# snphbaum/scikit-gpuppy

Measured on NVIDIA B200. Metric: fit_s_per_iter, lower is better.
Workload: dtype f64

## Files before the change

scikit-gpuppy_b200/csrc/gpk.cu:

```cuda
#include "../../include/gpk.h"
#include "../../include/gpk_test.h"

#include <climits>
#include <new>
#include <type_traits>
#include <vector>

#include "dgemm_dmma.cuh"
#include "factor.cuh"
#include "se_kernels.cuh"
#include "exact_kernels.cuh"
#include "periodic_kernels.cuh"

namespace gpk {
thread_local char g_err[512] = {0};
thread_local long g_launch_count = 0;
thread_local bool g_prof_on = false;
static thread_local std::vector<ProfPair> g_prof;
void prof_push(cudaEvent_t a, cudaEvent_t b) { g_prof.push_back(ProfPair{a, b}); }

struct Handle {
  int n = 0, d = 0, npad = 0;
  double *X = nullptr, *W = nullptr;
  bool own_X = false, own_W = false;
// ... 990 lines not shown
  if (npad % TILE) { snprintf(g_err, sizeof(g_err), "npad must be a multiple of 128"); return -2; }
  int* info_dev = nullptr;
  GPK_CUDA_OK(cudaMalloc((void**)&info_dev, sizeof(int)));
  set_int_kernel<<<1, 1, 0, st>>>(info_dev, INT_MAX);
  FactorCtx c{A, X, (long)ld, dL, info_dev, st};
  int rc = potrf_inv_node(c, 0, (int)npad);
  int info = 0;
  cudaError_t e = cudaMemcpyAsync(&info, info_dev, sizeof(int), cudaMemcpyDeviceToHost, st);
  if (e == cudaSuccess) e = cudaStreamSynchronize(st);
  cudaFree(info_dev);
  if (rc < 0) return rc;
  if (e != cudaSuccess) { snprintf(g_err, sizeof(g_err), "potrf_inv: %s", cudaGetErrorString(e)); return -1; }
  *info_host = (info == INT_MAX) ? 0 : info;
  return 0;
}

int gpk_test_oz_residues(const double* src, int64_t ld, int64_t rows, int64_t K, int trans, int lower, int moduli,
                         void* planes_out, double* scales_out, void* stream) {
  cudaStream_t st = reinterpret_cast<cudaStream_t>(stream);
  oz::Operand op;
  op.sl = reinterpret_cast<int8_t*>(planes_out); op.sc = scales_out;
  op.rows = (int)rows; op.K = (int)K; op.S = moduli;
  unsigned long long* mx = nullptr;
  GPK_CUDA_OK(cudaMalloc((void**)&mx, (size_t)rows * sizeof(unsigned long long)));
  int rc = oz::slice_operand(src, ld, trans, lower, op, mx, st);
  cudaError_t e = cudaStreamSynchronize(st);
  cudaFree(mx);
  if (rc < 0) return rc;
  if (e != cudaSuccess) { snprintf(g_err, sizeof(g_err), "oz_residues: %s", cudaGetErrorString(e)); return -1; }
  return 0;
}

int gpk_test_oz_gemm(const double* A, int64_t lda, int transA, int lowerA, const double* B, int64_t ldb, int transB,
                     int lowerB, double* C, int64_t ldc, int64_t M, int64_t N, int64_t K, double alpha, double beta,
                     int krange, int lower_only, int moduli, int64_t panel_rows, int reps, float* ms_out, void* stream) {
  cudaStream_t st = reinterpret_cast<cudaStream_t>(stream);
  oz::Operand a, b;
  a.rows = (int)M; a.K = (int)K; a.S = moduli;
  b.rows = (int)N; b.K = (int)K; b.S = moduli;
  unsigned long long* mx = nullptr;
  cudaEvent_t e0 = nullptr, e1 = nullptr, e2 = nullptr;
  int rc = 0;
  auto cleanup = [&]() {
    cudaFree(a.sl); cudaFree(a.sc); cudaFree(b.sl); cudaFree(b.sc); cudaFree(mx); cudaFree(a.out);
    if (e0) cudaEventDestroy(e0);
    if (e1) cudaEventDestroy(e1);
    if (e2) cudaEventDestroy(e2);
  };
#define OZ_OK(expr)                                                                         \
  do {                                                                                      \
    cudaError_t _e = (expr);                                                                \
    if (_e != cudaSuccess) {                                                                \
      snprintf(g_err, sizeof(g_err), "oz_gemm: %s -> %s", #expr, cudaGetErrorString(_e));   \
      cleanup();                                                                            \
      return -1;                                                                            \
    }                                                                                       \
  } while (0)
  OZ_OK(cudaMalloc((void**)&a.sl, oz::Operand::slice_bytes(a.rows, a.K, a.S)));
  OZ_OK(cudaMalloc((void**)&b.sl, oz::Operand::slice_bytes(b.rows, b.K, b.S)));
  OZ_OK(cudaMalloc((void**)&a.sc, (size_t)M * sizeof(double)));
  OZ_OK(cudaMalloc((void**)&b.sc, (size_t)N * sizeof(double)));
  OZ_OK(cudaMalloc((void**)&mx, (size_t)(M > N ? M : N) * sizeof(unsigned long long)));
  {
    const long prow = panel_rows > 0 ? round_up_l((long)panel_rows, 256) : round_up_l((long)M, 256);
    size_t want_out = (size_t)a.S * prow * round_up_l((long)N, 256);
    if (want_out > ((size_t)16 << 30)) want_out = (size_t)16 << 30;
    OZ_OK(cudaMalloc((void**)&a.out, want_out));
    a.out_cap = want_out;
  }
  OZ_OK(cudaEventCreate(&e0));
  OZ_OK(cudaEventCreate(&e1));
  OZ_OK(cudaEventCreate(&e2));
  OZ_OK(cudaEventRecord(e0, st));
  rc = oz::slice_operand(A, lda, transA, lowerA, a, mx, st);
  if (rc == 0) rc = oz::slice_operand(B, ldb, transB, lowerB, b, mx, st);
  if (rc < 0) { cleanup(); return rc; }
  OZ_OK(cudaEventRecord(e1, st));
  if (reps < 1) reps = 1;
  for (int r = 0; r < reps && rc == 0; ++r) rc = oz::gemm_sliced(a, b, C, ldc, alpha, beta, krange, lower_only, st);
  if (rc < 0) { cleanup(); return rc; }
  OZ_OK(cudaEventRecord(e2, st));
  OZ_OK(cudaStreamSynchronize(st));
  if (ms_out) {
    OZ_OK(cudaEventElapsedTime(&ms_out[0], e0, e1));
    OZ_OK(cudaEventElapsedTime(&ms_out[1], e1, e2));
    ms_out[1] /= reps;
  }
#undef OZ_OK
  cleanup();
  return 0;
}

int gpk_test_position_lock(int on) {
  if (on >= 0 && on <= 2) oz::g_position_lock = on;
  return oz::g_position_lock;
}

int gpk_test_overlap(int on) {
  if (on == 0 || on == 1) g_overlap_T = on;
  return g_overlap_T;
}

int gpk_profile(int on) {
  g_prof_on = on != 0;
  return 0;
}

int gpk_profile_read(double* gemm_ms, int64_t* gemm_launches, int64_t* all_launches, double* max_gemm_ms) {
  double total = 0.0, longest = 0.0;
  for (auto& p : g_prof) {
    float ms = 0.f;
    cudaError_t e = cudaEventSynchronize(p.b);
    if (e == cudaSuccess) e = cudaEventElapsedTime(&ms, p.a, p.b);
    cudaEventDestroy(p.a);
    cudaEventDestroy(p.b);
    if (e != cudaSuccess) {
      snprintf(g_err, sizeof(g_err), "gpk_profile_read: %s", cudaGetErrorString(e));
      g_prof.clear();
// ... 73 lines not shown
```

scikit-gpuppy_b200/csrc/oz_crt_planes.cuh:

```cuda

struct PlaneArgs {
  uint8_t* res; long res_ld; long res_plane;
  int M, N, K;
  int row_tile0;
  int krange, lower_only;
  int widen, band_cols;
  int nmod;
  unsigned int* phase;
  int* spill;
  int m[CRT_MAX_MODULI]; uint32_t magic[CRT_MAX_MODULI]; uint32_t u[CRT_MAX_MODULI];
};

constexpr int RECON_GROUPS = (CRT_MAX_MODULI + 3) / 4;

struct ReconArgs {
  const uint8_t* res; long res_ld; long res_plane;
  double* C; long ldc;
  const double* scA; const double* scB;
  double alpha, beta;
  int M, N, K;
  int row0;
  int krange, lower_only;
  int nmod;
  double p_scaled;
  double* colsq; double* pairdot; long ldo;
  uint32_t wp[2 * RECON_GROUPS][6];
};

constexpr int SPILL_SLOTS = 256;
constexpr int Q_BN = 256;
constexpr int Q_STAGES = 7;
constexpr int Q_STAGE_BYTES = 2 * TILE_BYTES;
constexpr int Q_SMEM_BYTES = Q_STAGES * Q_STAGE_BYTES + 1024 + 256;

__host__ __device__ __forceinline__ void planes_krange(int krange, int K, int bi2, int bx2, int& kb0, int& kb1) {
  kb0 = 0;
  kb1 = K / BK;
  switch (krange) {
    case K_UPTO_BJ: kb1 = (kb1 < 2 * bx2 + 2) ? kb1 : 2 * bx2 + 2; break;
    case K_FROM_BJ: kb0 = (kb1 < 2 * bx2) ? kb1 : 2 * bx2; break;
    case K_UPTO_BI: kb1 = (kb1 < 2 * bi2 + 2) ? kb1 : 2 * bi2 + 2; break;
    case K_FROM_BI: kb0 = (kb1 < 2 * bi2) ? kb1 : 2 * bi2; break;
    default: break;
  }
}

__global__ void __launch_bounds__(THREADS, 1)
// ... 24 lines not shown
    const int first = band * PLANES_BAND;
    const int cols = min(nx - first, PLANES_BAND);
    const int rem = pid - band * per_band;
    bx = first + rem % cols;
    by = rem / cols;
    band_lo = first;
    band_hi = first + cols - 1;
  }
  const int bi2 = by + p.row_tile0;
  const int bi = 2 * bi2 + pp;
  const int bjt = 2 * bx + pp;
  if (p.lower_only && 2 * bx > 2 * bi2 + 1) return;
  int kb0, kb1;
  planes_krange(p.krange, p.K, bi2, bx, kb0, kb1);
  if (kb1 <= kb0) return;
  if (p.widen) {
    const int kbt = p.K / BK;
    switch (p.krange) {
      case K_FROM_BI: case K_FROM_BJ: { const int u = min(kb0, 2 * band_lo); kb0 = max(u, kb0 - WIDEN_TILES); if (kb0 < 0) kb0 = 0; } break;
      case K_UPTO_BI: case K_UPTO_BJ: { const int u = max(kb1, min(kbt, 2 * band_hi + 2)); kb1 = min(u, kb1 + WIDEN_TILES); if (kb1 > kbt) kb1 = kbt; } break;
      default: break;
    }
  }
  const int nmod = p.nmod;

  const uint32_t raw = smem_u32(oz_smem_raw);
  uint8_t* smem = oz_smem_raw + ((1024u - (raw & 1023u)) & 1023u);
  uint64_t* bars = reinterpret_cast<uint64_t*>(smem + Q_STAGES * Q_STAGE_BYTES);
  uint64_t* full = bars;
  uint64_t* empty = bars + Q_STAGES;
  uint64_t* tmem_full = bars + 2 * Q_STAGES;
  uint64_t* tmem_empty = bars + 2 * Q_STAGES + 2;
  uint32_t* tmem_slot = reinterpret_cast<uint32_t*>(bars + 2 * Q_STAGES + 4);

  if (warp == 0 && lane == 0) {
    tma_prefetch_desc(&tmA);
    tma_prefetch_desc(&tmB);
  }
  if (warp == 1 && lane == 0) {
    for (int s = 0; s < Q_STAGES; ++s) {
      mbar_init(&full[s], 1);
      mbar_init(&empty[s], 1);
    }
    for (int b = 0; b < 2; ++b) {
      mbar_init(&tmem_full[b], 1);
      mbar_init(&tmem_empty[b], 2 * EPI_WARPS);
    }
// ... 71 lines not shown
            umma_i8_pair(acc, ad + (uint64_t)(k4 * 2), bd + (uint64_t)(k4 * 2), idesc, (kb > kbeg) | (k4 > 0));
          umma_commit_pair(&empty[stage], 3);
          if (++stage == Q_STAGES) { stage = 0; phase ^= 1u; }
        }
        umma_commit_pair(&tmem_full[buf], 3);
      }
    }
  } else {
    const int quad = warp & 3, half = (warp - 2) >> 2;
    const int row = quad * 32 + lane;
    const uint32_t lane_addr = tmem_base + ((uint32_t)(quad * 32) << 16);
    const long lrow = (long)by * (2 * BM) + pp * BM + row;
    uint8_t* dst0 = p.res + lrow * p.res_ld + (long)bx * Q_BN + half * 128;
    int4* sp = split ? reinterpret_cast<int4*>(p.spill + ((size_t)(smid % SPILL_SLOTS) * BM + row) * Q_BN + half * 128) : nullptr;
    for (int sg = 0; sg < nseg; ++sg) {
      const int i = SEG_MOD(sg);
      const bool spill_out = split && sg == 0, add_in = split && sg == nmod;
      const int buf = sg & 1;
      if (lane == 0) mbar_wait(&tmem_full[buf], (uint32_t)(sg >> 1) & 1u);
      __syncwarp();
      tc_fence_after();
      const int m = p.m[i];
      const int magic = (int)p.magic[i];
      const uint32_t u = p.u[i];
      uint8_t* dst = dst0 + (long)i * p.res_plane;
#pragma unroll
      for (int c = 0; c < 4; ++c) {
        uint32_t R[2][16];
        const uint32_t ta = lane_addr + (uint32_t)(buf * Q_BN + half * 128 + c * 32);
        tmem_ld16(ta, R[0]);
        tmem_ld16(ta + 16u, R[1]);
        tmem_ld_wait();
        if (c == 3) {
          tc_fence_before();
          __syncwarp();
          if (lane == 0) mbar_arrive_cluster(&tmem_empty[buf], rank & ~1u);
        }
        if (spill_out) {
#pragma unroll
          for (int x = 0; x < 8; ++x) {
            const uint32_t* r4 = &R[x >> 2][(x & 3) * 4];
            sp[c * 8 + x] = make_int4((int)r4[0], (int)r4[1], (int)r4[2], (int)r4[3]);
          }
          continue;
        }
        if (add_in) {
#pragma unroll
// ... 37 lines not shown
  uint32_t d;
  asm("dp2a.hi.u32.u32 %0, %1, %2, %3;" : "=r"(d) : "r"(a), "r"(b), "r"(c));
  return d;
}

template <int EPI, int NG>
__global__ void __launch_bounds__(256, 4) oz_crt_reconstruct_kernel(const __grid_constant__ ReconArgs p) {
  const int lane = threadIdx.x & 31, warp = threadIdx.x >> 5;
  const int bjc = blockIdx.x;
  const long lrow = (long)blockIdx.y * 8 + warp;
  const long grow = (long)p.row0 + lrow;
  const long gcol = (long)bjc * 128 + lane * 4;
  const int bi = (int)(grow >> 7), bi2 = (int)(grow >> 8), bx2 = bjc >> 1;
  if (EPI == OZ_EPI_STORE && p.lower_only && bjc > bi) return;
  int kb0, kb1;
  planes_krange(p.krange, p.K, bi2, bx2, kb0, kb1);
  const bool computed = (kb1 > kb0) && !(p.lower_only && 2 * bx2 > 2 * bi2 + 1);

  uint32_t acc[4][6];
#pragma unroll
  for (int x = 0; x < 4; ++x)
#pragma unroll
    for (int j = 0; j < 6; ++j) acc[x][j] = 0u;
  if (computed) {
    const uint8_t* src = p.res + lrow * p.res_ld + gcol;
    uint32_t q[NG * 4];
#pragma unroll
    for (int i = 0; i < NG * 4; ++i) {
      q[i] = (i < 4 * (NG - 1) || i < p.nmod) ? __ldcs(reinterpret_cast<const uint32_t*>(src)) : 0u;
      src += p.res_plane;
    }
#pragma unroll
    for (int g = 0; g < NG; ++g) {
      {
        const uint32_t ab_lo = __byte_perm(q[4 * g], q[4 * g + 1], 0x5140), ab_hi = __byte_perm(q[4 * g], q[4 * g + 1], 0x7362);
        const uint32_t cd_lo = __byte_perm(q[4 * g + 2], q[4 * g + 3], 0x5140),
                       cd_hi = __byte_perm(q[4 * g + 2], q[4 * g + 3], 0x7362);
        const uint32_t t[4] = {__byte_perm(ab_lo, cd_lo, 0x5410), __byte_perm(ab_lo, cd_lo, 0x7632),
                               __byte_perm(ab_hi, cd_hi, 0x5410), __byte_perm(ab_hi, cd_hi, 0x7632)};
#pragma unroll
        for (int e = 0; e < 4; ++e)
#pragma unroll
          for (int j = 0; j < 6; ++j) {
            uint32_t v = acc[e][j];
            v = dp2a_lo(p.wp[2 * g][j], t[e], v);
            v = dp2a_hi(p.wp[2 * g + 1][j], t[e], v);
            acc[e][j] = v;
          }
      }
    }
  }
  const bool row_ok = grow < p.M;
  const bool col_ok = gcol < p.N;
  const double sa = row_ok ? p.scA[grow] * p.p_scaled : 0.0;
  double v[4];
#pragma unroll
  for (int x = 0; x < 4; ++x) {
    const unsigned long long t0 = ((unsigned long long)acc[x][1] << 16) + acc[x][0];
    const unsigned long long t1 = ((unsigned long long)acc[x][3] << 16) + acc[x][2] + (t0 >> 32);
    const unsigned long long t2 = ((unsigned long long)acc[x][5] << 16) + acc[x][4] + (t1 >> 32);
    const long long hi = (long long)((t2 << 32) | (t1 & 0xffffffffull));
    const double frac = fma((double)hi, 4294967296.0, (double)(uint32_t)t0);
    v[x] = col_ok ? sa * p.scB[gcol + x] * frac : 0.0;
  }
  if (EPI == OZ_EPI_STORE) {
    if (row_ok && col_ok) {
      double* crow = p.C + grow * p.ldc + gcol;
#pragma unroll
      for (int x = 0; x < 4; x += 2) {
        double2 o;
        o.x = p.alpha * v[x];
        o.y = p.alpha * v[x + 1];
        if (p.beta != 0.0) {
          const double2 old = *reinterpret_cast<const double2*>(crow + x);
          o.x = fma(p.beta, old.x, o.x);
          o.y = fma(p.beta, old.y, o.y);
        }
// ... 26 lines not shown
```

scikit-gpuppy_b200/csrc/oz_gemm.cuh:

```cuda
#pragma once
#include <cuda.h>

#include "dgemm_dmma.cuh"
#include "oz_crt_tables.h"

namespace gpk {
namespace oz {

constexpr int BM = 128, BN = 128, BK = 128;
constexpr int TILE_BYTES = BM * BK;
constexpr int EPI_WARPS = 8;
constexpr int THREADS = 64 + EPI_WARPS * 32;
constexpr int TMEM_COLS = 512;

constexpr int OZ_EPI_STORE = 0;
constexpr int OZ_EPI_ROWSQ = 1;

__device__ __forceinline__ uint32_t smem_u32(const void* p) { return (uint32_t)__cvta_generic_to_shared(p); }

__device__ __forceinline__ void mbar_init(uint64_t* bar, uint32_t count) {
  asm volatile("mbarrier.init.shared::cta.b64 [%0], %1;" ::"r"(smem_u32(bar)), "r"(count) : "memory");
}
__device__ __forceinline__ void fence_barrier_init() {
  asm volatile("fence.mbarrier_init.release.cluster;" ::: "memory");
// ... 105 lines not shown

template <int TRANS>
__device__ __forceinline__ bool oz_valid(int r, int k, int lower) {
  if (!lower) return true;
  return TRANS ? ((r >> 7) <= (k >> 7)) : ((k >> 7) <= (r >> 7));
}
constexpr int WIDEN_MIN_K = 16384;
constexpr int PLANES_BAND = 4;
constexpr int WIDEN_TILES = 2 * (PLANES_BAND - 1);
inline int zero_fill_extra(int K) { return K >= WIDEN_MIN_K ? 1 + WIDEN_TILES : 1; }
template <int TRANS>
__device__ __forceinline__ bool oz_needed(int r, int k, int lower, int extra) {
  if (!lower) return true;
  return TRANS ? ((r >> 7) <= (k >> 7) + extra) : ((k >> 7) <= (r >> 7) + extra);
}

__device__ __forceinline__ size_t slice_offset(int rows, int K, int p, int r, int k) {
  const size_t tiles_per_plane = (size_t)(rows >> 7) * (size_t)(K >> 7);
  return (((size_t)p * tiles_per_plane + (size_t)(r >> 7) * (size_t)(K >> 7) + (size_t)(k >> 7)) << 14) +
         ((size_t)(r & 127) << 7) + (size_t)(k & 127);
}

__global__ void __launch_bounds__(256) oz_absmax_rows_kernel(const double* __restrict__ src, long ld, int K, int lower,
                                                             unsigned long long* __restrict__ mx) {
  __shared__ double red[8];
  const int r = blockIdx.x;
  const int kend = lower ? min(K, ((r >> 7) + 1) << 7) : K;
  const double* row = src + (long)r * ld;
  double m = 0.0;
  for (int k = threadIdx.x; k < kend; k += 256) m = fmax(m, fabs(row[k]));
#pragma unroll
  for (int o = 16; o > 0; o >>= 1) m = fmax(m, __shfl_xor_sync(0xffffffffu, m, o));
  if ((threadIdx.x & 31) == 0) red[threadIdx.x >> 5] = m;
  __syncthreads();
  if (threadIdx.x == 0) {
#pragma unroll
    for (int i = 0; i < 8; ++i) m = fmax(m, red[i]);
    mx[r] = (unsigned long long)__double_as_longlong(m);
  }
}
__global__ void __launch_bounds__(256) oz_absmax_cols_kernel(const double* __restrict__ src, long ld, int K, int lower,
                                                             unsigned long long* __restrict__ mx) {
  __shared__ double red[8][32];
  const int lane = threadIdx.x & 31, w = threadIdx.x >> 5;
  const int r = blockIdx.x * 32 + lane;
  const int k0 = blockIdx.y * 1024, k1 = min(K, k0 + 1024);
  const int kfirst = lower ? ((r >> 7) << 7) : 0;
  double m = 0.0;
  for (int k = k0 + w; k < k1; k += 8)
    if (k >= kfirst) m = fmax(m, fabs(src[(long)k * ld + r]));
  red[w][lane] = m;
  __syncthreads();
  if (w == 0) {
#pragma unroll
    for (int i = 1; i < 8; ++i) m = fmax(m, red[i][lane]);
    atomicMax(mx + r, (unsigned long long)__double_as_longlong(m));
  }
}

__device__ __forceinline__ int oz_row_exponent(unsigned long long bits) {
  const double m = __longlong_as_double((long long)bits);
  if (!(m > 0.0) || !isfinite(m)) return 0;
  int e = ilogb(m) + 1;
  if (e < -900) e = -900;
  return e;
}

__constant__ CrtModulus c_crt[CRT_MAX_MODULI];

inline int crt_upload_constants() {
  static bool done_on[GPK_MAX_DEVICES] = {};
  bool& done = done_on[current_device_slot()];
  if (done) return 0;
  const CrtSet& last = CRT_SETS[CRT_MAX_MODULI - CRT_MIN_MODULI];
  GPK_CUDA_OK(cudaMemcpyToSymbol(c_crt, last.mod, sizeof(CrtModulus) * CRT_MAX_MODULI));
  done = true;
  return 0;
}
inline const CrtSet& crt_set(int nmod) { return CRT_SETS[nmod - CRT_MIN_MODULI]; }
inline int crt_bits(int K, int nmod) {
  int b = (int)floor((crt_set(nmod).log2P - 1.0 - log2((double)K) - 1e-6) / 2.0);
  return b > 60 ? 60 : b;
}

inline int crt_moduli_for(int K, int want_bits) {
  for (int nmod = CRT_MIN_MODULI; nmod < CRT_MAX_MODULI; ++nmod)
    if (crt_bits(K, nmod) >= want_bits) return nmod;
  return CRT_MAX_MODULI;
}

__device__ __forceinline__ int dp4a_us(uint32_t a, uint32_t b, int c) {
  int d;
  asm("dp4a.u32.s32 %0, %1, %2, %3;" : "=r"(d) : "r"(a), "r"(b), "r"(c));
  return d;
}
__device__ __forceinline__ void oz_split(double x, double scale, uint32_t& lo, uint32_t& hi) {
  const unsigned long long X = (unsigned long long)(__double2ll_rn(x * scale) + (1ll << 62));
  lo = (uint32_t)X;
  hi = (uint32_t)(X >> 32);
}
__device__ __forceinline__ uint4 oz_residues16(const uint32_t (&lo)[16], const uint32_t (&hi)[16], int i) {
  const uint32_t dlo = c_crt[i].dlo, dhi = c_crt[i].dhi, m32c = c_crt[i].m32c;
  const int dinit = c_crt[i].dinit, m = c_crt[i].m, half = c_crt[i].half;
  uint32_t w[4];
#pragma unroll
  for (int g = 0; g < 4; ++g) {
    uint32_t word = 0u;
#pragma unroll
    for (int b = 0; b < 4; ++b) {
      const int e = g * 4 + b;
      const int t = dp4a_us(lo[e], dlo, dp4a_us(hi[e], dhi, dinit));
      const uint32_t q = __umulhi((uint32_t)t, m32c);
      const int r = t - (int)q * m - half;
      word = __byte_perm(word, (uint32_t)r, 0x3210u ^ ((0x4u ^ (uint32_t)b) << (4 * b)));
    }
    w[g] = word;
  }
  return make_uint4(w[0], w[1], w[2], w[3]);
}

__global__ void __launch_bounds__(256) oz_residue_rows_kernel(const double* __restrict__ src, long ld, int rows, int K,
                                                              int lower, int nmod, int bits, int extra,
                                                              const unsigned long long* __restrict__ mx,
                                                              int8_t* __restrict__ sl, double* __restrict__ sc) {
  const long idx = (long)blockIdx.x * 256 + threadIdx.x;
  const int cpr = K >> 4;
  if (idx >= (long)rows * cpr) return;
  const int r = (int)(idx / cpr), ch = (int)(idx % cpr);
  const int e = oz_row_exponent(mx[r]);
  if (ch == 0) sc[r] = ldexp(1.0, e - bits);
  const double scale = ldexp(1.0, bits - e);
  const int k0 = ch << 4;
  if (!oz_needed<0>(r, k0, lower, extra)) return;
  uint32_t lo[16], hi[16];
  if (oz_valid<0>(r, k0, lower)) {
    const double2* s2 = reinterpret_cast<const double2*>(src + (long)r * ld + k0);
#pragma unroll
    for (int i = 0; i < 8; ++i) {
      const double2 v = s2[i];
      oz_split(v.x, scale, lo[2 * i], hi[2 * i]);
      oz_split(v.y, scale, lo[2 * i + 1], hi[2 * i + 1]);
    }
  } else {
#pragma unroll
    for (int i = 0; i < 16; ++i) oz_split(0.0, scale, lo[i], hi[i]);
  }
  for (int p = 0; p < nmod; ++p)
    *reinterpret_cast<uint4*>(sl + slice_offset(rows, K, p, r, k0)) = oz_residues16(lo, hi, p);
}

__global__ void __launch_bounds__(256) oz_residue_cols_kernel(const double* __restrict__ src, long ld, int rows, int K,
                                                              int lower, int nmod, int bits, int extra,
                                                              const unsigned long long* __restrict__ mx,
                                                              int8_t* __restrict__ sl, double* __restrict__ sc) {
  const int lane = threadIdx.x & 31, w = threadIdx.x >> 5;
  const int r = blockIdx.x * 32 + lane;
  const int k0 = (blockIdx.y * 8 + w) * 16;
  if (k0 >= K) return;
  const int e = oz_row_exponent(mx[r]);
  if (k0 == 0) sc[r] = ldexp(1.0, e - bits);
  const double scale = ldexp(1.0, bits - e);
  if (!oz_needed<1>(r, k0, lower, extra)) return;
  uint32_t lo[16], hi[16];
  const bool valid = oz_valid<1>(r, k0, lower);
#pragma unroll
  for (int i = 0; i < 16; ++i) oz_split(valid ? src[(long)(k0 + i) * ld + r] : 0.0, scale, lo[i], hi[i]);
  for (int p = 0; p < nmod; ++p)
    *reinterpret_cast<uint4*>(sl + slice_offset(rows, K, p, r, k0)) = oz_residues16(lo, hi, p);
}

#include "oz_crt_planes.cuh"

typedef CUresult (*EncodeTiledFn)(CUtensorMap*, CUtensorMapDataType, cuuint32_t, void*, const cuuint64_t*, const cuuint64_t*,
                                  const cuuint32_t*, const cuuint32_t*, CUtensorMapInterleave, CUtensorMapSwizzle,
                                  CUtensorMapL2promotion, CUtensorMapFloatOOBfill);

inline EncodeTiledFn encode_fn() {
  static EncodeTiledFn fn = [] {
    void* f = nullptr;
    cudaDriverEntryPointQueryResult q;
    if (cudaGetDriverEntryPoint("cuTensorMapEncodeTiled", &f, cudaEnableDefault, &q) != cudaSuccess ||
        q != cudaDriverEntryPointSuccess)
      f = nullptr;
    return reinterpret_cast<EncodeTiledFn>(f);
  }();
  return fn;
}

inline int make_tmap(CUtensorMap* tm, const int8_t* base, int rows, int K, int S, int box_rows = BM) {
  EncodeTiledFn enc = encode_fn();
  if (!enc) {
    snprintf(g_err, sizeof(g_err), "cuTensorMapEncodeTiled entry point not available");
    return -1;
  }
  const cuuint64_t kbs = (cuuint64_t)(K / BK), rts = (cuuint64_t)(rows / BM);
  cuuint64_t dims[5] = {(cuuint64_t)BK, (cuuint64_t)BM, kbs, rts, (cuuint64_t)S};
  cuuint64_t strides[4] = {(cuuint64_t)BK, (cuuint64_t)TILE_BYTES, (cuuint64_t)TILE_BYTES * kbs,
                           (cuuint64_t)TILE_BYTES * kbs * rts};
  cuuint32_t box[5] = {(cuuint32_t)BK, (cuuint32_t)box_rows, 1, 1, 1};
  cuuint32_t estr[5] = {1, 1, 1, 1, 1};
  CUresult r = enc(tm, CU_TENSOR_MAP_DATA_TYPE_UINT8, 5, const_cast<int8_t*>(base), dims, strides, box, estr,
                   CU_TENSOR_MAP_INTERLEAVE_NONE, CU_TENSOR_MAP_SWIZZLE_128B, CU_TENSOR_MAP_L2_PROMOTION_L2_256B,
                   CU_TENSOR_MAP_FLOAT_OOB_FILL_NONE);
  if (r != CUDA_SUCCESS) {
    snprintf(g_err, sizeof(g_err), "cuTensorMapEncodeTiled failed (%d) rows=%d K=%d S=%d", (int)r, rows, K, S);
    return -1;
  }
  return 0;
}
struct Operand {
  int8_t* sl = nullptr;
  double* sc = nullptr;
  int rows = 0, K = 0, S = 0;
  int bits = 0;
  uint8_t* out = nullptr;
  size_t out_cap = 0;
  static size_t slice_bytes(int rows, int K, int S) { return (size_t)S * rows * K; }
};

inline int slice_operand(const double* src, long ld, int trans, int lower, Operand& op, unsigned long long* mx,
                         cudaStream_t st) {
  if (op.rows % BM || op.K % BK || op.S < CRT_MIN_MODULI || op.S > CRT_MAX_MODULI) {
    snprintf(g_err, sizeof(g_err), "slice_operand: bad shape rows=%d K=%d moduli=%d", op.rows, op.K, op.S);
    return -2;
  }
  GPK_TRY(crt_upload_constants());
  op.bits = crt_bits(op.K, op.S);
  if (!trans) {
    oz_absmax_rows_kernel<<<op.rows, 256, 0, st>>>(src, ld, op.K, lower, mx);
    GPK_LAUNCH_OK();
    const long chunks = (long)op.rows * (op.K >> 4);
    oz_residue_rows_kernel<<<(unsigned)((chunks + 255) / 256), 256, 0, st>>>(src, ld, op.rows, op.K, lower, op.S,
                                                                            op.bits, zero_fill_extra(op.K), mx, op.sl, op.sc);
    GPK_LAUNCH_OK();
  } else {
    GPK_CUDA_OK(cudaMemsetAsync(mx, 0, (size_t)op.rows * sizeof(unsigned long long), st));
    dim3 g1(op.rows / 32, (op.K + 1023) / 1024);
    oz_absmax_cols_kernel<<<g1, 256, 0, st>>>(src, ld, op.K, lower, mx);
    GPK_LAUNCH_OK();
    dim3 g2(op.rows / 32, (op.K + 127) / 128);
    oz_residue_cols_kernel<<<g2, 256, 0, st>>>(src, ld, op.rows, op.K, lower, op.S, op.bits, zero_fill_extra(op.K), mx, op.sl, op.sc);
    GPK_LAUNCH_OK();
  }
  return 0;
}

thread_local int g_position_lock = 2;

inline int gemm_sliced(const Operand& A, const Operand& B, double* C, long ldc, double alpha, double beta, int krange,
                       int lower_only, cudaStream_t st, int epi = OZ_EPI_STORE, double* colsq = nullptr,
                       double* pairdot = nullptr, long ldo = 0) {
  if (A.K != B.K || A.S != B.S) {
    snprintf(g_err, sizeof(g_err), "gemm_sliced: operand mismatch K %d/%d moduli %d/%d", A.K, B.K, A.S, B.S);
    return -2;
  }
  if (A.bits != B.bits || A.bits != crt_bits(A.K, A.S)) {
    snprintf(g_err, sizeof(g_err), "gemm_sliced: operand widths %d/%d do not match K=%d", A.bits, B.bits, A.K);
    return -2;
  }
  const long Nc = ((long)B.rows + Q_BN - 1) / Q_BN * Q_BN;
  const size_t per_row = (size_t)A.S * (size_t)Nc;
  const long panel = (long)(A.out_cap / per_row) / 256 * 256;
  if (!A.out || panel < 256) {
    snprintf(g_err, sizeof(g_err), "gemm_sliced: the residue-plane buffer (%zu bytes) cannot hold a 256-row panel of %ld columns",
             A.out_cap, Nc);
    return -4;
  }
  static bool configured_on[GPK_MAX_DEVICES] = {};
  bool& configured = configured_on[current_device_slot()];
  if (!configured) {
    GPK_CUDA_OK(cudaFuncSetAttribute(oz_crt_planes_kernel, cudaFuncAttributeMaxDynamicSharedMemorySize, Q_SMEM_BYTES));
    configured = true;
  }
  CUtensorMap tmA, tmB;
  GPK_TRY(make_tmap(&tmA, A.sl, A.rows, A.K, A.S, BM));
  GPK_TRY(make_tmap(&tmB, B.sl, B.rows, B.K, B.S, BM));
  const CrtSet& cs = crt_set(A.S);
  PlaneArgs g;
  memset(&g, 0, sizeof(g));
  g.res = A.out; g.res_ld = Nc;
  g.M = A.rows; g.N = B.rows; g.K = A.K; g.krange = krange; g.lower_only = lower_only; g.nmod = A.S;
  g.widen = (g_position_lock >= 2 && A.K >= WIDEN_MIN_K &&
             (krange == K_FROM_BI || krange == K_UPTO_BI || krange == K_FROM_BJ || krange == K_UPTO_BJ)) ? 1 : 0;
  g.band_cols = (g.widen && (krange == K_FROM_BJ || krange == K_UPTO_BJ)) ? 1 : 0;
  ReconArgs r;
  memset(&r, 0, sizeof(r));
  r.res = A.out; r.res_ld = Nc;
  r.C = C; r.ldc = ldc; r.scA = A.sc; r.scB = B.sc; r.alpha = alpha; r.beta = beta;
  r.M = A.rows; r.N = B.rows; r.K = A.K; r.krange = krange; r.lower_only = lower_only; r.nmod = A.S;
  r.p_scaled = cs.p_scaled;
  r.colsq = colsq; r.pairdot = pairdot; r.ldo = ldo;
  for (int i = 0; i < A.S; ++i) {
    g.m[i] = cs.mod[i].m; g.magic[i] = cs.mod[i].magic; g.u[i] = (uint32_t)cs.mod[i].u;
    const uint32_t w[3] = {cs.mod[i].w0, cs.mod[i].w1, cs.mod[i].w2};
    for (int j = 0; j < 6; ++j) {
      const uint32_t limb = (w[j >> 1] >> (16 * (j & 1))) & 0xffffu;
      r.wp[i >> 1][j] |= limb << (16 * (i & 1));
    }
  }
  static unsigned int* phase_dev_on[GPK_MAX_DEVICES] = {};
  unsigned int*& phase_dev = phase_dev_on[current_device_slot()];
  if (!phase_dev) GPK_CUDA_OK(cudaMalloc((void**)&phase_dev, 64 * sizeof(unsigned int)));
  static thread_local int phase_next = 0;
  static int* spill_dev_on[GPK_MAX_DEVICES] = {};
  int*& spill_dev = spill_dev_on[current_device_slot()];
  if (!spill_dev) GPK_CUDA_OK(cudaMalloc((void**)&spill_dev, (size_t)SPILL_SLOTS * BM * Q_BN * sizeof(int)));
  g.spill = g_position_lock ? spill_dev : nullptr;
  cudaEvent_t e0 = nullptr, e1 = nullptr;
  if (g_prof_on) {
    GPK_CUDA_OK(cudaEventCreate(&e0));
    GPK_CUDA_OK(cudaEventCreate(&e1));
    GPK_CUDA_OK(cudaEventRecord(e0, st));
  }
  for (long row0 = 0; row0 < A.rows; row0 += panel) {
    const long rows = (A.rows - row0 < panel) ? A.rows - row0 : panel;
    const long rows_pad = (rows + 255) / 256 * 256;
// ... 22 lines not shown
    GPK_LAUNCH_OK();
    long ncol_blocks = B.rows / 128;
    if (lower_only && (row0 + rows) / 128 < ncol_blocks) ncol_blocks = (row0 + rows) / 128;
    dim3 rg((unsigned)ncol_blocks, (unsigned)(rows / 8));
    const int ng = (A.S + 3) / 4;
    const bool store = epi == OZ_EPI_STORE;
    auto kernel = (ng <= 2) ? (store ? oz_crt_reconstruct_kernel<OZ_EPI_STORE, 2> : oz_crt_reconstruct_kernel<OZ_EPI_ROWSQ, 2>)
                : (ng == 3) ? (store ? oz_crt_reconstruct_kernel<OZ_EPI_STORE, 3> : oz_crt_reconstruct_kernel<OZ_EPI_ROWSQ, 3>)
                : (ng == 4) ? (store ? oz_crt_reconstruct_kernel<OZ_EPI_STORE, 4> : oz_crt_reconstruct_kernel<OZ_EPI_ROWSQ, 4>)
                            : (store ? oz_crt_reconstruct_kernel<OZ_EPI_STORE, 5> : oz_crt_reconstruct_kernel<OZ_EPI_ROWSQ, 5>);
    kernel<<<rg, 256, 0, st>>>(r);
    GPK_LAUNCH_OK();
  }
  if (g_prof_on) {
    GPK_CUDA_OK(cudaEventRecord(e1, st));
    prof_push(e0, e1);
  }
  return 0;
}

struct Workspace {
  int8_t* buf = nullptr; size_t cap = 0, top = 0;
  double* sc = nullptr; size_t sc_cap = 0, sc_top = 0;
  unsigned long long* mx = nullptr; size_t mx_cap = 0;
  uint8_t* out = nullptr; size_t out_cap = 0;
  int S = CRT_MIN_MODULI;
  int min_dim = 2048;
  void reset() { top = 0; sc_top = 0; }
  Operand alloc(int rows, int K) {
    Operand op;
    const size_t bytes = Operand::slice_bytes(rows, K, S);
    if (top + bytes > cap || sc_top + (size_t)rows > sc_cap || (size_t)rows > mx_cap) return op;
    op.sl = buf + top; op.sc = sc + sc_top; op.rows = rows; op.K = K; op.S = S;
    op.out = out; op.out_cap = out_cap;
    top += bytes; sc_top += (size_t)rows;
    return op;
  }
  int ensure_out(size_t bytes) {
    if (bytes <= out_cap) return 0;
    if (out) cudaFree(out);
    out = nullptr; out_cap = 0;
    if (cudaMalloc((void**)&out, bytes) != cudaSuccess) { cudaGetLastError(); out = nullptr; return -1; }
    out_cap = bytes;
    return 0;
  }
  int ensure(size_t bytes, size_t rows_total, size_t rows_max) {
    if (bytes > cap) {
      if (buf) cudaFree(buf);
      buf = nullptr; cap = 0;
      if (cudaMalloc((void**)&buf, bytes) != cudaSuccess) { cudaGetLastError(); buf = nullptr; return -1; }
      cap = bytes;
    }
    if (rows_total > sc_cap) {
      if (sc) cudaFree(sc);
      sc = nullptr; sc_cap = 0;
      if (cudaMalloc((void**)&sc, rows_total * sizeof(double)) != cudaSuccess) { cudaGetLastError(); return -1; }
      sc_cap = rows_total;
    }
    if (rows_max > mx_cap) {
      if (mx) cudaFree(mx);
      mx = nullptr; mx_cap = 0;
      if (cudaMalloc((void**)&mx, rows_max * sizeof(unsigned long long)) != cudaSuccess) { cudaGetLastError(); return -1; }
      mx_cap = rows_max;
    }
    return 0;
  }
  void release() {
    if (buf) cudaFree(buf);
    if (sc) cudaFree(sc);
    if (mx) cudaFree(mx);
    if (out) cudaFree(out);
    buf = nullptr; sc = nullptr; mx = nullptr; out = nullptr; cap = sc_cap = mx_cap = out_cap = 0;
  }
};

inline int gemm_f64(Workspace& ws, const double* A, long lda, int transA, int lowerA, int M, const double* B, long ldb,
                    int transB, int lowerB, int N, int K, double* C, long ldc, double alpha, double beta, int krange,
                    int lower_only, cudaStream_t st) {
  ws.reset();
  Operand a = ws.alloc(M, K);
  const bool same = (A == B && lda == ldb && transA == transB && lowerA == lowerB && M == N);
  Operand b = same ? a : ws.alloc(N, K);
  if (!a.sl || !b.sl) {
    snprintf(g_err, sizeof(g_err), "gemm_f64: residue workspace too small for %d x %d and %d x %d operands", M, K, N, K);
    return -4;
  }
  GPK_TRY(slice_operand(A, lda, transA, lowerA, a, ws.mx, st));
  if (same) b = a;
  else GPK_TRY(slice_operand(B, ldb, transB, lowerB, b, ws.mx, st));
  return gemm_sliced(a, b, C, ldc, alpha, beta, krange, lower_only, st);
}

}
}
```

scikit-gpuppy_b200/skgpuppy/_native.py:

```python
import ctypes
import os

import numpy as np

_HERE = os.path.dirname(os.path.abspath(__file__))
_LIB_PATH = os.path.join(_HERE, "libgpk.so")
_lib = None

c_double_p = ctypes.POINTER(ctypes.c_double)
c_int_p = ctypes.POINTER(ctypes.c_int)
i64 = ctypes.c_int64
vp = ctypes.c_void_p

SIGNATURES = {
    "gpk_version": (ctypes.c_int, []),
    "gpk_last_error": (ctypes.c_char_p, []),
    "gpk_npad": (i64, [i64]),
    "gpk_create": (ctypes.c_int, [i64, i64, vp, vp, ctypes.POINTER(vp)]),
    "gpk_destroy": (ctypes.c_int, [vp]),
    "gpk_set_stream": (ctypes.c_int, [vp, vp]),
    "gpk_set_data": (ctypes.c_int, [vp, vp, vp]),
    "gpk_kernel_matrix": (ctypes.c_int, [vp, i64, vp, i64, i64, c_double_p, ctypes.c_int, vp, i64, vp]),
    "gpk_factorize": (ctypes.c_int, [vp, c_double_p, ctypes.c_int]),
    "gpk_factorize_matrix": (ctypes.c_int, [vp, vp, i64, ctypes.c_int]),
# ... 6 lines not shown
    "gpk_solve_residual": (ctypes.c_int, [vp, c_double_p]),
    "gpk_get_alpha": (ctypes.c_int, [vp, vp]),
    "gpk_import_state": (ctypes.c_int, [vp, c_double_p, vp, ctypes.c_int]),
    "gpk_predict": (ctypes.c_int, [vp, vp, i64, ctypes.c_double, vp, vp, ctypes.c_int]),
    "gpk_predict_cross": (ctypes.c_int, [vp, vp, i64, i64, vp, ctypes.c_double, vp, vp]),
    "gpk_propagate_ga": (ctypes.c_int, [vp, vp, vp, i64, ctypes.c_int, ctypes.c_double, vp, vp]),
    "gpk_propagate_ga_parts": (ctypes.c_int, [vp, vp, vp, i64, ctypes.c_int, vp, vp]),
    "gpk_propagate_exact": (ctypes.c_int, [vp, vp, vp, vp, vp, i64, ctypes.c_double, vp, vp]),
    "gpk_set_kernel": (ctypes.c_int, [vp, ctypes.c_int]),
    "gpk_kernel_matrix_periodic": (ctypes.c_int, [vp, i64, vp, i64, i64, c_double_p, ctypes.c_int, vp, i64, vp]),
    "gpk_set_route": (ctypes.c_int, [vp, ctypes.c_int, i64, ctypes.c_int, i64]),
    "gpk_get_route": (ctypes.c_int, [vp, c_int_p]),
    "gpk_set_batch_rows": (ctypes.c_int, [vp, i64]),
}

TEST_SIGNATURES = {
    "gpk_test_potrf_inv": (ctypes.c_int, [vp, vp, i64, i64, vp, c_int_p, vp]),
    "gpk_test_oz_residues": (ctypes.c_int, [vp, i64, i64, i64, ctypes.c_int, ctypes.c_int, ctypes.c_int, vp, vp, vp]),
    "gpk_test_oz_gemm": (ctypes.c_int, [vp, i64, ctypes.c_int, ctypes.c_int, vp, i64, ctypes.c_int, ctypes.c_int, vp, i64,
                                        i64, i64, i64, ctypes.c_double, ctypes.c_double, ctypes.c_int, ctypes.c_int,
                                        ctypes.c_int, i64, ctypes.c_int, ctypes.POINTER(ctypes.c_float), vp]),
    "gpk_test_overlap": (ctypes.c_int, [ctypes.c_int]),
    "gpk_test_position_lock": (ctypes.c_int, [ctypes.c_int]),
    "gpk_profile": (ctypes.c_int, [ctypes.c_int]),
    "gpk_profile_read": (ctypes.c_int, [c_double_p, ctypes.POINTER(i64), ctypes.POINTER(i64), c_double_p]),
    "gpk_microbench_i8": (ctypes.c_int, [i64, ctypes.c_double, c_double_p]),
}


class GpkError(RuntimeError):
    pass


def lib_path():
    return _LIB_PATH


def load():
    global _lib
    if _lib is not None:
        return _lib
    if not os.path.exists(_LIB_PATH):
        raise GpkError(
            "libgpk.so not found at %s: build it with `python scikit-gpuppy_b200/build_native.py` "
            "(there is no CPU fallback)" % _LIB_PATH)
    lib = ctypes.CDLL(_LIB_PATH)
# ... 43 lines not shown
```

Before: 0.3090.

## Drop one CRT modulus per GEMM when operand row norms bound the product range

While slicing operands, per-row sums of squared coarse magnitudes are accumulated. Before each Ozaki GEMM, a single-block kernel takes the max of these over A and B. If their product (a Cauchy-Schwarz bound on the dot products) fits under the smaller modulus set's range, the plane and reconstruction kernels read a device-side modulus count and skip the last modulus, switching to the matching CRT constants. This saves one int8 GEMM plane plus its reconstruction when data allows. It costs extra atomics in the residue kernels and one extra tiny launch per GEMM, and correctness depends on the bound.

```diff
diff --git a/scikit-gpuppy_b200/csrc/gpk.cu b/scikit-gpuppy_b200/csrc/gpk.cu
--- a/scikit-gpuppy_b200/csrc/gpk.cu
+++ b/scikit-gpuppy_b200/csrc/gpk.cu
@@ -1036,7 +1036,8 @@
   op.sl = reinterpret_cast<int8_t*>(planes_out); op.sc = scales_out;
   op.rows = (int)rows; op.K = (int)K; op.S = moduli;
   unsigned long long* mx = nullptr;
-  GPK_CUDA_OK(cudaMalloc((void**)&mx, (size_t)rows * sizeof(unsigned long long)));
+  GPK_CUDA_OK(cudaMalloc((void**)&mx, 2 * (size_t)rows * sizeof(unsigned long long)));
+  op.rsq = mx + rows;
   int rc = oz::slice_operand(src, ld, trans, lower, op, mx, st);
   cudaError_t e = cudaStreamSynchronize(st);
   cudaFree(mx);
@@ -1056,7 +1057,8 @@
   cudaEvent_t e0 = nullptr, e1 = nullptr, e2 = nullptr;
   int rc = 0;
   auto cleanup = [&]() {
-    cudaFree(a.sl); cudaFree(a.sc); cudaFree(b.sl); cudaFree(b.sc); cudaFree(mx); cudaFree(a.out);
+    cudaFree(a.sl); cudaFree(a.sc); cudaFree(a.rsq); cudaFree(b.sl); cudaFree(b.sc); cudaFree(b.rsq); cudaFree(mx);
+    cudaFree(a.out);
     if (e0) cudaEventDestroy(e0);
     if (e1) cudaEventDestroy(e1);
     if (e2) cudaEventDestroy(e2);
@@ -1074,6 +1076,8 @@
   OZ_OK(cudaMalloc((void**)&b.sl, oz::Operand::slice_bytes(b.rows, b.K, b.S)));
   OZ_OK(cudaMalloc((void**)&a.sc, (size_t)M * sizeof(double)));
   OZ_OK(cudaMalloc((void**)&b.sc, (size_t)N * sizeof(double)));
+  OZ_OK(cudaMalloc((void**)&a.rsq, (size_t)M * sizeof(unsigned long long)));
+  OZ_OK(cudaMalloc((void**)&b.rsq, (size_t)N * sizeof(unsigned long long)));
   OZ_OK(cudaMalloc((void**)&mx, (size_t)(M > N ? M : N) * sizeof(unsigned long long)));
   {
     const long prow = panel_rows > 0 ? round_up_l((long)panel_rows, 256) : round_up_l((long)M, 256);
@@ -1108,6 +1112,21 @@
 int gpk_test_position_lock(int on) {
   if (on >= 0 && on <= 2) oz::g_position_lock = on;
   return oz::g_position_lock;
+}
+
+int gpk_test_crt_range(int on) {
+  if (on == 0 || on == 1) oz::g_crt_range = on;
+  return oz::g_crt_range;
+}
+
+int64_t gpk_test_crt_counts(int* counts_host, int64_t cap) {
+  const long n = oz::g_crt_counts;
+  oz::g_crt_counts = 0;
+  if (n == 0) return 0;
+  GPK_CUDA_OK(cudaDeviceSynchronize());
+  const long kept = n < oz::CRT_COUNT_LOG ? n : oz::CRT_COUNT_LOG;
+  for (long i = 0; i < kept && i < cap; ++i) counts_host[i] = oz::g_crt_count_log[i];
+  return n;
 }
 
 int gpk_test_overlap(int on) {
diff --git a/scikit-gpuppy_b200/csrc/oz_crt_planes.cuh b/scikit-gpuppy_b200/csrc/oz_crt_planes.cuh
--- a/scikit-gpuppy_b200/csrc/oz_crt_planes.cuh
+++ b/scikit-gpuppy_b200/csrc/oz_crt_planes.cuh
@@ -5,10 +5,12 @@
   int row_tile0;
   int krange, lower_only;
   int widen, band_cols;
-  int nmod;
+  int S;
+  const int* nmod;
   unsigned int* phase;
   int* spill;
-  int m[CRT_MAX_MODULI]; uint32_t magic[CRT_MAX_MODULI]; uint32_t u[CRT_MAX_MODULI];
+  int m[CRT_MAX_MODULI]; uint32_t magic[CRT_MAX_MODULI];
+  uint32_t u[2][CRT_MAX_MODULI];
 };
 
 constexpr int RECON_GROUPS = (CRT_MAX_MODULI + 3) / 4;
@@ -21,8 +23,8 @@
   int M, N, K;
   int row0;
   int krange, lower_only;
-  int nmod;
-  double p_scaled;
+  int S; const int* nmod;
+  double p_scaled[2];
   double* colsq; double* pairdot; long ldo;
   uint32_t wp[2 * RECON_GROUPS][6];
 };
@@ -93,7 +95,8 @@
       default: break;
     }
   }
-  const int nmod = p.nmod;
+  const int nmod = *p.nmod;
+  const uint32_t* u_set = p.u[nmod == p.S ? 0 : 1];
 
   const uint32_t raw = smem_u32(oz_smem_raw);
   uint8_t* smem = oz_smem_raw + ((1024u - (raw & 1023u)) & 1023u);
@@ -211,7 +214,7 @@
       tc_fence_after();
       const int m = p.m[i];
       const int magic = (int)p.magic[i];
-      const uint32_t u = p.u[i];
+      const uint32_t u = u_set[i];
       uint8_t* dst = dst0 + (long)i * p.res_plane;
 #pragma unroll
       for (int c = 0; c < 4; ++c) {
@@ -295,12 +298,13 @@
   for (int x = 0; x < 4; ++x)
 #pragma unroll
     for (int j = 0; j < 6; ++j) acc[x][j] = 0u;
+  const int nmod = *p.nmod;
   if (computed) {
     const uint8_t* src = p.res + lrow * p.res_ld + gcol;
     uint32_t q[NG * 4];
 #pragma unroll
     for (int i = 0; i < NG * 4; ++i) {
-      q[i] = (i < 4 * (NG - 1) || i < p.nmod) ? __ldcs(reinterpret_cast<const uint32_t*>(src)) : 0u;
+      q[i] = (i < 4 * (NG - 1) || i < nmod) ? __ldcs(reinterpret_cast<const uint32_t*>(src)) : 0u;
       src += p.res_plane;
     }
 #pragma unroll
@@ -325,7 +329,7 @@
   }
   const bool row_ok = grow < p.M;
   const bool col_ok = gcol < p.N;
-  const double sa = row_ok ? p.scA[grow] * p.p_scaled : 0.0;
+  const double sa = row_ok ? p.scA[grow] * p.p_scaled[nmod == p.S ? 0 : 1] : 0.0;
   double v[4];
 #pragma unroll
   for (int x = 0; x < 4; ++x) {
diff --git a/scikit-gpuppy_b200/csrc/oz_gemm.cuh b/scikit-gpuppy_b200/csrc/oz_gemm.cuh
--- a/scikit-gpuppy_b200/csrc/oz_gemm.cuh
+++ b/scikit-gpuppy_b200/csrc/oz_gemm.cuh
@@ -1,5 +1,7 @@
 #pragma once
 #include <cuda.h>
+
+#include <atomic>
 
 #include "dgemm_dmma.cuh"
 #include "oz_crt_tables.h"
@@ -151,7 +153,8 @@
 }
 
 __global__ void __launch_bounds__(256) oz_absmax_rows_kernel(const double* __restrict__ src, long ld, int K, int lower,
-                                                             unsigned long long* __restrict__ mx) {
+                                                             unsigned long long* __restrict__ mx,
+                                                             unsigned long long* __restrict__ rsq) {
   __shared__ double red[8];
   const int r = blockIdx.x;
   const int kend = lower ? min(K, ((r >> 7) + 1) << 7) : K;
@@ -166,10 +169,12 @@
 #pragma unroll
     for (int i = 0; i < 8; ++i) m = fmax(m, red[i]);
     mx[r] = (unsigned long long)__double_as_longlong(m);
+    rsq[r] = 0ull;
   }
 }
 __global__ void __launch_bounds__(256) oz_absmax_cols_kernel(const double* __restrict__ src, long ld, int K, int lower,
-                                                             unsigned long long* __restrict__ mx) {
+                                                             unsigned long long* __restrict__ mx,
+                                                             unsigned long long* __restrict__ rsq) {
   __shared__ double red[8][32];
   const int lane = threadIdx.x & 31, w = threadIdx.x >> 5;
   const int r = blockIdx.x * 32 + lane;
@@ -184,6 +189,7 @@
 #pragma unroll
     for (int i = 1; i < 8; ++i) m = fmax(m, red[i][lane]);
     atomicMax(mx + r, (unsigned long long)__double_as_longlong(m));
+    if (blockIdx.y == 0) rsq[r] = 0ull;
   }
 }
 
@@ -223,10 +229,27 @@
   asm("dp4a.u32.s32 %0, %1, %2, %3;" : "=r"(d) : "r"(a), "r"(b), "r"(c));
   return d;
 }
-__device__ __forceinline__ void oz_split(double x, double scale, uint32_t& lo, uint32_t& hi) {
-  const unsigned long long X = (unsigned long long)(__double2ll_rn(x * scale) + (1ll << 62));
+__host__ __device__ __forceinline__ int rsq_shift(int bits) { return bits > 16 ? bits - 16 : 0; }
+__device__ __forceinline__ void oz_split(double x, double scale, int sh, uint32_t& lo, uint32_t& hi,
+                                         unsigned long long& sq) {
+  const long long v = __double2ll_rn(x * scale);
+  const unsigned long long a = (unsigned long long)(v < 0 ? -v : v);
+  const uint32_t c = (uint32_t)((a + ((1ull << sh) - 1ull)) >> sh);
+  sq += (unsigned long long)c * c;
+  const unsigned long long X = (unsigned long long)(v + (1ll << 62));
   lo = (uint32_t)X;
   hi = (uint32_t)(X >> 32);
+}
+__device__ __forceinline__ void oz_rsq_add_warp(unsigned long long v, int r, int rows, unsigned long long* rsq) {
+  const int lane = threadIdx.x & 31;
+#pragma unroll
+  for (int o = 1; o < 32; o <<= 1) {
+    const unsigned long long vo = __shfl_down_sync(0xffffffffu, v, o);
+    const int ro = __shfl_down_sync(0xffffffffu, r, o);
+    if (lane + o < 32 && ro == r) v += vo;
+  }
+  const int rprev = __shfl_up_sync(0xffffffffu, r, 1);
+  if ((lane == 0 || rprev != r) && r < rows && v) atomicAdd(rsq + r, v);
 }
 __device__ __forceinline__ uint4 oz_residues16(const uint32_t (&lo)[16], const uint32_t (&hi)[16], int i) {
   const uint32_t dlo = c_crt[i].dlo, dhi = c_crt[i].dhi, m32c = c_crt[i].m32c;
@@ -251,51 +274,71 @@
 __global__ void __launch_bounds__(256) oz_residue_rows_kernel(const double* __restrict__ src, long ld, int rows, int K,
                                                               int lower, int nmod, int bits, int extra,
                                                               const unsigned long long* __restrict__ mx,
-                                                              int8_t* __restrict__ sl, double* __restrict__ sc) {
+                                                              int8_t* __restrict__ sl, double* __restrict__ sc,
+                                                              unsigned long long* __restrict__ rsq) {
   const long idx = (long)blockIdx.x * 256 + threadIdx.x;
   const int cpr = K >> 4;
-  if (idx >= (long)rows * cpr) return;
-  const int r = (int)(idx / cpr), ch = (int)(idx % cpr);
-  const int e = oz_row_exponent(mx[r]);
-  if (ch == 0) sc[r] = ldexp(1.0, e - bits);
-  const double scale = ldexp(1.0, bits - e);
-  const int k0 = ch << 4;
-  if (!oz_needed<0>(r, k0, lower, extra)) return;
-  uint32_t lo[16], hi[16];
-  if (oz_valid<0>(r, k0, lower)) {
-    const double2* s2 = reinterpret_cast<const double2*>(src + (long)r * ld + k0);
-#pragma unroll
-    for (int i = 0; i < 8; ++i) {
-      const double2 v = s2[i];
-      oz_split(v.x, scale, lo[2 * i], hi[2 * i]);
-      oz_split(v.y, scale, lo[2 * i + 1], hi[2 * i + 1]);
+  const int sh = rsq_shift(bits);
+  const bool in = idx < (long)rows * cpr;
+  const int r = in ? (int)(idx / cpr) : rows, ch = in ? (int)(idx % cpr) : 0;
+  unsigned long long sq = 0ull;
+  if (in) {
+    const int e = oz_row_exponent(mx[r]);
+    if (ch == 0) sc[r] = ldexp(1.0, e - bits);
+    const double scale = ldexp(1.0, bits - e);
+    const int k0 = ch << 4;
+    if (oz_needed<0>(r, k0, lower, extra)) {
+      uint32_t lo[16], hi[16];
+      if (oz_valid<0>(r, k0, lower)) {
+        const double2* s2 = reinterpret_cast<const double2*>(src + (long)r * ld + k0);
+#pragma unroll
+        for (int i = 0; i < 8; ++i) {
+          const double2 v = s2[i];
+          oz_split(v.x, scale, sh, lo[2 * i], hi[2 * i], sq);
+          oz_split(v.y, scale, sh, lo[2 * i + 1], hi[2 * i + 1], sq);
+        }
+      } else {
+#pragma unroll
+        for (int i = 0; i < 16; ++i) oz_split(0.0, scale, sh, lo[i], hi[i], sq);
+      }
+      for (int p = 0; p < nmod; ++p)
+        *reinterpret_cast<uint4*>(sl + slice_offset(rows, K, p, r, k0)) = oz_residues16(lo, hi, p);
     }
-  } else {
-#pragma unroll
-    for (int i = 0; i < 16; ++i) oz_split(0.0, scale, lo[i], hi[i]);
-  }
-  for (int p = 0; p < nmod; ++p)
-    *reinterpret_cast<uint4*>(sl + slice_offset(rows, K, p, r, k0)) = oz_residues16(lo, hi, p);
+  }
+  oz_rsq_add_warp(sq, r, rows, rsq);
 }
 
 __global__ void __launch_bounds__(256) oz_residue_cols_kernel(const double* __restrict__ src, long ld, int rows, int K,
                                                               int lower, int nmod, int bits, int extra,
                                                               const unsigned long long* __restrict__ mx,
-                                                              int8_t* __restrict__ sl, double* __restrict__ sc) {
+                                                              int8_t* __restrict__ sl, double* __restrict__ sc,
+                                                              unsigned long long* __restrict__ rsq) {
+  __shared__ unsigned long long red[8][32];
   const int lane = threadIdx.x & 31, w = threadIdx.x >> 5;
   const int r = blockIdx.x * 32 + lane;
   const int k0 = (blockIdx.y * 8 + w) * 16;
-  if (k0 >= K) return;
-  const int e = oz_row_exponent(mx[r]);
-  if (k0 == 0) sc[r] = ldexp(1.0, e - bits);
-  const double scale = ldexp(1.0, bits - e);
-  if (!oz_needed<1>(r, k0, lower, extra)) return;
-  uint32_t lo[16], hi[16];
-  const bool valid = oz_valid<1>(r, k0, lower);
-#pragma unroll
-  for (int i = 0; i < 16; ++i) oz_split(valid ? src[(long)(k0 + i) * ld + r] : 0.0, scale, lo[i], hi[i]);
-  for (int p = 0; p < nmod; ++p)
-    *reinterpret_cast<uint4*>(sl + slice_offset(rows, K, p, r, k0)) = oz_residues16(lo, hi, p);
+  const int sh = rsq_shift(bits);
+  unsigned long long sq = 0ull;
+  if (k0 < K) {
+    const int e = oz_row_exponent(mx[r]);
+    if (k0 == 0) sc[r] = ldexp(1.0, e - bits);
+    const double scale = ldexp(1.0, bits - e);
+    if (oz_needed<1>(r, k0, lower, extra)) {
+      uint32_t lo[16], hi[16];
+      const bool valid = oz_valid<1>(r, k0, lower);
+#pragma unroll
+      for (int i = 0; i < 16; ++i) oz_split(valid ? src[(long)(k0 + i) * ld + r] : 0.0, scale, sh, lo[i], hi[i], sq);
+      for (int p = 0; p < nmod; ++p)
+        *reinterpret_cast<uint4*>(sl + slice_offset(rows, K, p, r, k0)) = oz_residues16(lo, hi, p);
+    }
+  }
+  red[w][lane] = sq;
+  __syncthreads();
+  if (w == 0) {
+#pragma unroll
+    for (int i = 1; i < 8; ++i) sq += red[i][lane];
+    if (sq) atomicAdd(rsq + r, sq);
+  }
 }
 
 #include "oz_crt_planes.cuh"
@@ -340,6 +383,7 @@
 struct Operand {
   int8_t* sl = nullptr;
   double* sc = nullptr;
+  unsigned long long* rsq = nullptr;
   int rows = 0, K = 0, S = 0;
   int bits = 0;
   uint8_t* out = nullptr;
@@ -356,25 +400,51 @@
   GPK_TRY(crt_upload_constants());
   op.bits = crt_bits(op.K, op.S);
   if (!trans) {
-    oz_absmax_rows_kernel<<<op.rows, 256, 0, st>>>(src, ld, op.K, lower, mx);
+    oz_absmax_rows_kernel<<<op.rows, 256, 0, st>>>(src, ld, op.K, lower, mx, op.rsq);
     GPK_LAUNCH_OK();
     const long chunks = (long)op.rows * (op.K >> 4);
     oz_residue_rows_kernel<<<(unsigned)((chunks + 255) / 256), 256, 0, st>>>(src, ld, op.rows, op.K, lower, op.S,
-                                                                            op.bits, zero_fill_extra(op.K), mx, op.sl, op.sc);
+                                                                            op.bits, zero_fill_extra(op.K), mx, op.sl, op.sc,
+                                                                            op.rsq);
     GPK_LAUNCH_OK();
   } else {
     GPK_CUDA_OK(cudaMemsetAsync(mx, 0, (size_t)op.rows * sizeof(unsigned long long), st));
     dim3 g1(op.rows / 32, (op.K + 1023) / 1024);
-    oz_absmax_cols_kernel<<<g1, 256, 0, st>>>(src, ld, op.K, lower, mx);
+    oz_absmax_cols_kernel<<<g1, 256, 0, st>>>(src, ld, op.K, lower, mx, op.rsq);
     GPK_LAUNCH_OK();
     dim3 g2(op.rows / 32, (op.K + 127) / 128);
-    oz_residue_cols_kernel<<<g2, 256, 0, st>>>(src, ld, op.rows, op.K, lower, op.S, op.bits, zero_fill_extra(op.K), mx, op.sl, op.sc);
+    oz_residue_cols_kernel<<<g2, 256, 0, st>>>(src, ld, op.rows, op.K, lower, op.S, op.bits, zero_fill_extra(op.K), mx, op.sl, op.sc,
+                                               op.rsq);
     GPK_LAUNCH_OK();
   }
   return 0;
 }
 
 thread_local int g_position_lock = 2;
+thread_local int g_crt_range = 1;
+constexpr int CRT_COUNT_LOG = 1 << 16;
+thread_local int* g_crt_count_log = nullptr;
+thread_local long g_crt_counts = 0;
+
+__global__ void __launch_bounds__(1024) oz_crt_count_kernel(const unsigned long long* __restrict__ ra, int na,
+                                                            const unsigned long long* __restrict__ rb, int nb, double thr,
+                                                            int S, int* __restrict__ nmod) {
+  __shared__ unsigned long long red[2][32];
+  unsigned long long ma = 0ull, mb = 0ull;
+  for (int i = threadIdx.x; i < na; i += 1024) ma = max(ma, ra[i]);
+  for (int i = threadIdx.x; i < nb; i += 1024) mb = max(mb, rb[i]);
+#pragma unroll
+  for (int o = 16; o > 0; o >>= 1) {
+    ma = max(ma, __shfl_xor_sync(0xffffffffu, ma, o));
+    mb = max(mb, __shfl_xor_sync(0xffffffffu, mb, o));
+  }
+  if ((threadIdx.x & 31) == 0) { red[0][threadIdx.x >> 5] = ma; red[1][threadIdx.x >> 5] = mb; }
+  __syncthreads();
+  if (threadIdx.x == 0) {
+    for (int i = 1; i < 32; ++i) { ma = max(ma, red[0][i]); mb = max(mb, red[1][i]); }
+    *nmod = __dmul_ru((double)ma, (double)mb) < thr ? S - 1 : S;
+  }
+}
 
 inline int gemm_sliced(const Operand& A, const Operand& B, double* C, long ldc, double alpha, double beta, int krange,
                        int lower_only, cudaStream_t st, int epi = OZ_EPI_STORE, double* colsq = nullptr,
@@ -405,10 +475,27 @@
   GPK_TRY(make_tmap(&tmA, A.sl, A.rows, A.K, A.S, BM));
   GPK_TRY(make_tmap(&tmB, B.sl, B.rows, B.K, B.S, BM));
   const CrtSet& cs = crt_set(A.S);
+  const bool may_drop = g_crt_range && A.S - 1 >= CRT_MIN_MODULI;
+  const CrtSet& cs1 = crt_set(may_drop ? A.S - 1 : A.S);
+  const double thr = may_drop ? exp2(2.0 * (cs1.log2P - 1.0) - 4.0 * rsq_shift(A.bits)) * (1.0 - 0x1p-18) : 0.0;
+  constexpr int NMOD_SLOTS = 1024;
+  static int* nmod_dev_on[GPK_MAX_DEVICES] = {};
+  static std::atomic<unsigned int> nmod_next_on[GPK_MAX_DEVICES];
+  int*& nmod_dev = nmod_dev_on[current_device_slot()];
+  if (!nmod_dev) GPK_CUDA_OK(cudaMalloc((void**)&nmod_dev, NMOD_SLOTS * sizeof(int)));
+  int* nmod = nmod_dev + nmod_next_on[current_device_slot()].fetch_add(1u) % NMOD_SLOTS;
+  oz_crt_count_kernel<<<1, 1024, 0, st>>>(A.rsq, A.rows, B.rsq, B.rows, thr, A.S, nmod);
+  GPK_LAUNCH_OK();
+  if (g_prof_on) {
+    if (!g_crt_count_log) GPK_CUDA_OK(cudaHostAlloc((void**)&g_crt_count_log, CRT_COUNT_LOG * sizeof(int), cudaHostAllocPortable));
+    if (g_crt_counts < CRT_COUNT_LOG)
+      GPK_CUDA_OK(cudaMemcpyAsync(g_crt_count_log + g_crt_counts, nmod, sizeof(int), cudaMemcpyDeviceToHost, st));
+    ++g_crt_counts;
+  }
   PlaneArgs g;
   memset(&g, 0, sizeof(g));
   g.res = A.out; g.res_ld = Nc;
-  g.M = A.rows; g.N = B.rows; g.K = A.K; g.krange = krange; g.lower_only = lower_only; g.nmod = A.S;
+  g.M = A.rows; g.N = B.rows; g.K = A.K; g.krange = krange; g.lower_only = lower_only; g.S = A.S; g.nmod = nmod;
   g.widen = (g_position_lock >= 2 && A.K >= WIDEN_MIN_K &&
              (krange == K_FROM_BI || krange == K_UPTO_BI || krange == K_FROM_BJ || krange == K_UPTO_BJ)) ? 1 : 0;
   g.band_cols = (g.widen && (krange == K_FROM_BJ || krange == K_UPTO_BJ)) ? 1 : 0;
@@ -416,11 +503,12 @@
   memset(&r, 0, sizeof(r));
   r.res = A.out; r.res_ld = Nc;
   r.C = C; r.ldc = ldc; r.scA = A.sc; r.scB = B.sc; r.alpha = alpha; r.beta = beta;
-  r.M = A.rows; r.N = B.rows; r.K = A.K; r.krange = krange; r.lower_only = lower_only; r.nmod = A.S;
-  r.p_scaled = cs.p_scaled;
+  r.M = A.rows; r.N = B.rows; r.K = A.K; r.krange = krange; r.lower_only = lower_only; r.S = A.S; r.nmod = nmod;
+  r.p_scaled[0] = cs.p_scaled; r.p_scaled[1] = cs1.p_scaled;
   r.colsq = colsq; r.pairdot = pairdot; r.ldo = ldo;
   for (int i = 0; i < A.S; ++i) {
-    g.m[i] = cs.mod[i].m; g.magic[i] = cs.mod[i].magic; g.u[i] = (uint32_t)cs.mod[i].u;
+    g.m[i] = cs.mod[i].m; g.magic[i] = cs.mod[i].magic;
+    g.u[0][i] = (uint32_t)cs.mod[i].u; g.u[1][i] = (uint32_t)cs1.mod[i].u;
     const uint32_t w[3] = {cs.mod[i].w0, cs.mod[i].w1, cs.mod[i].w2};
     for (int j = 0; j < 6; ++j) {
       const uint32_t limb = (w[j >> 1] >> (16 * (j & 1))) & 0xffffu;
@@ -489,6 +577,7 @@
 struct Workspace {
   int8_t* buf = nullptr; size_t cap = 0, top = 0;
   double* sc = nullptr; size_t sc_cap = 0, sc_top = 0;
+  unsigned long long* rsq = nullptr;
   unsigned long long* mx = nullptr; size_t mx_cap = 0;
   uint8_t* out = nullptr; size_t out_cap = 0;
   int S = CRT_MIN_MODULI;
@@ -498,7 +587,7 @@
     Operand op;
     const size_t bytes = Operand::slice_bytes(rows, K, S);
     if (top + bytes > cap || sc_top + (size_t)rows > sc_cap || (size_t)rows > mx_cap) return op;
-    op.sl = buf + top; op.sc = sc + sc_top; op.rows = rows; op.K = K; op.S = S;
+    op.sl = buf + top; op.sc = sc + sc_top; op.rsq = rsq + sc_top; op.rows = rows; op.K = K; op.S = S;
     op.out = out; op.out_cap = out_cap;
     top += bytes; sc_top += (size_t)rows;
     return op;
@@ -520,8 +609,10 @@
     }
     if (rows_total > sc_cap) {
       if (sc) cudaFree(sc);
-      sc = nullptr; sc_cap = 0;
+      if (rsq) cudaFree(rsq);
+      sc = nullptr; rsq = nullptr; sc_cap = 0;
       if (cudaMalloc((void**)&sc, rows_total * sizeof(double)) != cudaSuccess) { cudaGetLastError(); return -1; }
+      if (cudaMalloc((void**)&rsq, rows_total * sizeof(unsigned long long)) != cudaSuccess) { cudaGetLastError(); return -1; }
       sc_cap = rows_total;
     }
     if (rows_max > mx_cap) {
@@ -535,9 +626,10 @@
   void release() {
     if (buf) cudaFree(buf);
     if (sc) cudaFree(sc);
+    if (rsq) cudaFree(rsq);
     if (mx) cudaFree(mx);
     if (out) cudaFree(out);
-    buf = nullptr; sc = nullptr; mx = nullptr; out = nullptr; cap = sc_cap = mx_cap = out_cap = 0;
+    buf = nullptr; sc = nullptr; rsq = nullptr; mx = nullptr; out = nullptr; cap = sc_cap = mx_cap = out_cap = 0;
   }
 };
 
diff --git a/scikit-gpuppy_b200/skgpuppy/_native.py b/scikit-gpuppy_b200/skgpuppy/_native.py
--- a/scikit-gpuppy_b200/skgpuppy/_native.py
+++ b/scikit-gpuppy_b200/skgpuppy/_native.py
@@ -52,6 +52,8 @@
                                         ctypes.c_int, i64, ctypes.c_int, ctypes.POINTER(ctypes.c_float), vp]),
     "gpk_test_overlap": (ctypes.c_int, [ctypes.c_int]),
     "gpk_test_position_lock": (ctypes.c_int, [ctypes.c_int]),
+    "gpk_test_crt_range": (ctypes.c_int, [ctypes.c_int]),
+    "gpk_test_crt_counts": (i64, [c_int_p, i64]),
     "gpk_profile": (ctypes.c_int, [ctypes.c_int]),
     "gpk_profile_read": (ctypes.c_int, [c_double_p, ctypes.POINTER(i64), ctypes.POINTER(i64), c_double_p]),
     "gpk_microbench_i8": (ctypes.c_int, [i64, ctypes.c_double, c_double_p]),
```

Result: faster. 0.2989, median of 6 (-3.2%).
